# AnimatedRNG/alphazero-rs

Hardware: AMD Instinct MI355X
Metric: selfplay_games_per_sec (higher is better)
Workload: dtype bf16

## Files before the change

alphazero-rs_amd/csrc/az_engine.hip:

```cpp
#include "../../include/az_engine.h"

#include <dlfcn.h>
#include <unistd.h>
#include <rccl/rccl.h>

#include <algorithm>
#include <array>
#include <atomic>
#include <chrono>
#include <cstdio>
#include <cstring>
#include <map>
#include <memory>
#include <mutex>
#include <string>
#include <vector>

#include "az_combine.h"
#include "az_local_comm.h"
#include "az_net.h"
#include "az_train.h"
#include "az_tree.h"

using namespace az;
// ... 917 lines not shown
        const bool eps = is("root_noise_eps_e6");
        if (eps ? (value < 0 || value > 1000000) : (value < 50000 || value > 100000000))
            return fail(e, AZ_ERR_BAD_ARGUMENT, eps ? "root_noise_eps_e6 must be in 0 .. 1000000" : "root_noise_alpha_e6 must be in 50000 .. 100000000");
        if (e->sp_session) return fail(e, AZ_ERR_BAD_ARGUMENT, "root noise cannot change while a self-play session is open");
        (eps ? e->root_noise_eps_e6 : e->root_noise_alpha_e6) = value;
        return AZ_OK;
    }
    if (is("playout_cap_sims") || is("playout_cap_full_e6")) {
        const bool sims = is("playout_cap_sims");
        if (value < 0 || value > (sims ? PLAYOUT_CAP_MAX_SIMS : PLAYOUT_CAP_E6))
            return fail(e, AZ_ERR_BAD_ARGUMENT, sims ? "playout_cap_sims must be in 0 .. 65535" : "playout_cap_full_e6 must be in 0 .. 1000000");
        if (e->sp_session) return fail(e, AZ_ERR_BAD_ARGUMENT, "the playout cap cannot change while a self-play session is open");
        (sims ? e->playout_cap_sims : e->playout_cap_full_e6) = value;
        return AZ_OK;
    }
    if (is("forced_playouts_k_e6") || is("policy_prune")) {
        const bool k = is("forced_playouts_k_e6");
        if (value < 0 || value > (k ? FORCED_K_E6_MAX : 1))
            return fail(e, AZ_ERR_BAD_ARGUMENT, k ? "forced_playouts_k_e6 must be in 0 .. 16000000" : "policy_prune must be 0 or 1");
        if (e->sp_session) return fail(e, AZ_ERR_BAD_ARGUMENT, "forced playouts cannot change while a self-play session is open");
        (k ? e->forced_playouts_k_e6 : e->policy_prune) = value;
        return AZ_OK;
    }
    if (is("arena_opening_plies")) {
        if (value < 0 || value > OPENING_MAX_PLIES || (value & 1)) return fail(e, AZ_ERR_BAD_ARGUMENT, "arena_opening_plies must be 0 or an even value in 2 .. 12");
        e->arena_opening_plies = value;
        return AZ_OK;
    }
    if (is("conv3_small") && (value == 0 || value == 1)) { e->netopt.conv3_small = (int)value; return AZ_OK; }
    if (is("conv3_tail") && (value == 0 || value == 1)) { e->netopt.conv3_tail = (int)value; return AZ_OK; }
    if (is("ring_packed") && (value == 0 || value == 1)) { e->netopt.ring_packed = (int)value; return AZ_OK; }
    if (is("conv3_planes") && (value == 0 || value == 1)) { e->netopt.conv3_planes = (int)value; return AZ_OK; }
    if (is("conv3_wreg") && (value == 0 || value == 1)) { e->netopt.conv3_wreg = (int)value; return AZ_OK; }
    if (is("narrow_rows") && value >= 0 && value <= 65536) { e->netopt.narrow_rows = (int)value; return AZ_OK; }
    if (is("tree_block4") && (value == 0 || value == 1)) { e->tree_block4 = (int)value; return AZ_OK; }
    if (is("dedup_stats") && (value == 0 || value == 1)) { e->dedup_stats = (int)value; return AZ_OK; }
    if (is("profile_every") && value >= 1 && value <= 1000000) { e->profile_every = (int)value; return AZ_OK; }
    if (is("profile") && (value == 0 || value == 1)) { e->prof.on = value != 0; return AZ_OK; }
    if (is("search_graph") && value >= 0 && value <= 1000 && value % 2 == 0) { e->search_graph = (int)value; return AZ_OK; }
    if (is("search_graph_rows") && value >= 0 && value <= 1000000) { e->search_graph_rows = (int)value; return AZ_OK; }
    if (is("selfplay_async") && (value == 0 || value == 1)) { e->selfplay_async = (int)value; return AZ_OK; }
    if (is("selfplay_async_launches") && value >= 1 && value <= 8) { e->selfplay_async_launches = (int)value; return AZ_OK; }
    if (is("selfplay_async_iters") && value >= 2 && value <= 64) { e->selfplay_async_iters = (int)value; return AZ_OK; }
    if (is("fused_search") && (value == 0 || value == 1)) { e->fused_search = (int)value; return AZ_OK; }
    if (is("eval_dedup") && value >= 0 && value <= 2) { e->eval_dedup = (int)value; return AZ_OK; }
    if (is("eval_cache_log2") && (value == 0 || (value >= 10 && value <= 30))) { e->eval_cache_log2 = (int)value; return AZ_OK; }
    if (is("eval_cache_max_stones") && value >= 0 && value <= 42) { e->eval_cache_max_stones = (int)value; return AZ_OK; }
    if (is("eval_cache_persist") && (value == 0 || value == 1)) { e->eval_cache_persist = (int)value; return AZ_OK; }
    if (is("train_epochs") && value >= 1 && value <= 100000) { e->train_epochs = (int)value; return AZ_OK; }
    if (is("train_batch") && value >= 2 && value <= TRAIN_MAX_BATCH) { e->train_batch = (int)value; return AZ_OK; }
    if (is("train_seed")) { e->train_seed = (uint64_t)value; return AZ_OK; }
    if (is("train_graph") && (value == 0 || value == 1)) { e->train_graph = (int)value; if (e->trainer) trainer_set_graph(e->trainer, value != 0); return AZ_OK; }
    if (is("train_gemm3_ring") && (value == 0 || value == 1)) { e->train_gemm3_ring = (int)value; if (e->trainer) trainer_set_gemm3_ring(e->trainer, value != 0); return AZ_OK; }
    if (is("train_fwd_x3") && (value == 0 || value == 1)) { e->train_fwd_x3 = (int)value; if (e->trainer) trainer_set_fwd_x3(e->trainer, value != 0); return AZ_OK; }
    if (is("train_wgrad_tr") && (value == 0 || value == 1)) { e->train_wgrad_tr = (int)value; if (e->trainer) trainer_set_wgrad_tr(e->trainer, value != 0); return AZ_OK; }
    if (is("train_implicit") && (value == 0 || value == 1)) { e->train_implicit = (int)value; if (e->trainer) trainer_set_implicit(e->trainer, value != 0); return AZ_OK; }
    if (is("train_fork") && (value == 0 || value == 1)) {
        e->train_fork = (int)value;
        if (e->trainer) { (void)hipSetDevice(e->device); trainer_set_fork(e->trainer, value != 0); }
        return AZ_OK;
    }
    if (is("train_gemm") && (value == 0 || value == 1)) { e->train_gemm = (int)value; if (e->trainer) trainer_set_gemm(e->trainer, (int)value); return AZ_OK; }
    if (is("train_fwd_dma") && (value == 0 || value == 1)) { e->train_fwd_dma = (int)value; if (e->trainer) trainer_set_fwd_dma(e->trainer, value != 0); return AZ_OK; }
    if (is("train_lr_e9") && value > 0) { e->hyper.lr = (float)((double)value * 1e-9); return AZ_OK; }
    if (is("train_dropout_e6") && value >= 0 && value < 1000000) { e->hyper.dropout = (float)((double)value * 1e-6); return AZ_OK; }
#ifdef AZ_DIAG
// ... 1606 lines not shown
```

alphazero-rs_amd/csrc/az_net.h:

```cpp
#pragma once
#include "az_tree.h"

namespace az {

struct ConvNet;
struct NetWorkspace;

struct Layout {
    int C;
    int64_t conv_w[4], conv_b[4], conv_bn[4], fc_w[2], fc_b[2], fc_bn[2], pi_w, pi_b, v_w, v_b, total;
    explicit Layout(int c) : C(c) {
        int64_t o = 0;
        for (int l = 0; l < 4; ++l) {
            int cin = l == 0 ? 2 : C;
            conv_w[l] = o; o += 9ll * cin * C;
            conv_b[l] = o; o += C;
            conv_bn[l] = o; o += 4ll * C;
        }
        const int fin[2] = {6 * C, 1024}, fout[2] = {1024, 512};
        for (int l = 0; l < 2; ++l) {
            fc_w[l] = o; o += (int64_t)fin[l] * fout[l];
            fc_b[l] = o; o += fout[l];
            fc_bn[l] = o; o += 4ll * fout[l];
        }
// ... 3 lines not shown
    }
};


struct NetProfile {
    double conv2_ms = 0, conv2_flops = 0, total_ms = 0, total_flops = 0;
    double conv3_ms = 0, conv3_flops = 0;
    double conv4_ms = 0, conv4_flops = 0;
    double fc_ms = 0, fc_flops = 0;
    double rows = 0;
    double conv2_bytes = 0;
    uint64_t launches = 0;
};

void launch_net_fixture(const EvalBatch& eb, int kind, uint64_t salt, hipStream_t s);

ConvNet* convnet_create(int channels, const char** err);
void convnet_destroy(ConvNet* n);
NetWorkspace* netws_create(int channels, int max_batch, const char** err);
void netws_destroy(NetWorkspace* ws);
int64_t convnet_param_count(int channels);
bool convnet_set_params(ConvNet* n, const float* host_params, int64_t count);
bool convnet_get_params(const ConvNet* n, float* host_params, int64_t count);
void convnet_init_random(ConvNet* n, uint64_t seed);
void netws_resolve_profile(NetWorkspace* ws, NetProfile* prof);
bool netws_conv3_accounting(NetWorkspace* ws, unsigned long long out[2], bool reset);
struct NetOptions {
    int conv2_table = 1;
    int conv3_small = 1;
    int conv3_planes = 1;
    int ring_packed = 1;
    int conv3_tail = 1;
    int conv3_wreg = 1;
    int net_fp8 = 0;
    int narrow_rows = 32;
    int gemm_variant = 5;
    int conv1_table = 1;
    int conv2_pipe = 1;
    int conv3_pipe = 1;
    int conv3_ring = 0;
    int conv4_big = 0;
    int fc_ring = 1;
    int ring_tile[6] = {0, 0, 0, 0, 0, 0};
};
bool netws_read_clock_stamps(NetWorkspace* ws, unsigned long long* out2048);
long long netws_read_conv3_out(NetWorkspace* ws, int rows, void* out);
#ifdef AZ_DIAG
long long netws_read_act(NetWorkspace* ws, int layer, int rows, void* out);
long long convnet_read_conv_table(const ConvNet* n, int which, int first_row, int n_rows, void* out);
#endif
long long netws_read_conv3_out_fp8(NetWorkspace* ws, int rows, void* out);
long long netws_read_conv2_out_fp8(NetWorkspace* ws, int rows, void* out);
unsigned long long netws_fp8_skinny_launches(const NetWorkspace* ws);
bool convnet_build_fp8(ConvNet* n, NetWorkspace* ws, hipStream_t s);
bool convnet_fp8_scales(const ConvNet* n, float out[2]);
bool convnet_prepare(NetWorkspace* ws, const NetOptions& opt);
void convnet_forward(ConvNet* n, NetWorkspace* ws, const EvalBatch& eb, int n_rows_hint, int n_rows_typ, hipStream_t s, NetProfile* prof,
                     const NetOptions& opt);

}
```

alphazero-rs_amd/csrc/az_net.hip:

```cpp
#include "az_net.h"
#include "az_fp8.h"

#include <algorithm>
#include <cmath>
#include <cstring>
#include <vector>

namespace az {

constexpr int ACTIONS = ConnectFour::ACTIONS;

typedef __bf16 bf16x8 __attribute__((ext_vector_type(8)));
typedef float f32x4 __attribute__((ext_vector_type(4)));
typedef int i32x4 __attribute__((ext_vector_type(4)));
typedef int i32x8 __attribute__((ext_vector_type(8)));

__global__ void k_net_fixture(EvalBatch eb, int kind, uint64_t salt) {
    uint32_t i = blockIdx.x * blockDim.x + threadIdx.x;
    if (i >= *eb.n) return;
    float pi[ACTIONS], v;
    if (kind == 0) {
#pragma unroll
        for (int a = 0; a < ACTIONS; ++a) pi[a] = __fdiv_rn(1.0f, 7.0f);
        v = 1.0f;
// ... 511 lines not shown
    constexpr int BMAX = NS == 2 ? 192 : 128;
    __shared__ __attribute__((aligned(16))) unsigned char smem[NS * (BMAX * 128 + 16384)];
    const int M = (int)(*d.n_dev) * d.rows_per_sample;
    if (M <= d.m_min || (d.m_hi > 0 && M > d.m_hi)) return;
    const int bm = __builtin_amdgcn_readfirstlane(ring_pick_bm(M, d.N / GBN, NS, d.tap_w > 1));
    if constexpr (NS == 2) {
        if (bm == 96) gemm_ring_body<2, 96>(d, smem, M);
        else if (bm == 160) gemm_ring_body<2, 160>(d, smem, M);
        else if (bm == 192) gemm_ring_body<2, 192>(d, smem, M);
        else gemm_ring_body<2, 128>(d, smem, M);
    } else {
        if (bm == 64) gemm_ring_body<4, 64>(d, smem, M);
        else if (bm == 96) gemm_ring_body<4, 96>(d, smem, M);
        else gemm_ring_body<4, 128>(d, smem, M);
    }
}

template <int LAYER, int NS, int F8>
__global__ __launch_bounds__(256, (NS <= 2 ? 2 : 1)) void k_gemm_ring_f8(const GemmDesc d) {
    constexpr int BMAX = NS == 2 ? 192 : 128;
    __shared__ __attribute__((aligned(16))) unsigned char smem[NS * (BMAX * 128 + 16384)];
    const int M = (int)(*d.n_dev) * d.rows_per_sample;
    if (M <= d.m_min) return;
    const int bm = __builtin_amdgcn_readfirstlane(ring_pick_bm(M, d.N / GBN, NS, true));
    if constexpr (NS == 2) {
        if (bm == 96) gemm_ring_body<2, 96, F8>(d, smem, M);
        else if (bm == 160) gemm_ring_body<2, 160, F8>(d, smem, M);
        else if (bm == 192) gemm_ring_body<2, 192, F8>(d, smem, M);
        else gemm_ring_body<2, 128, F8>(d, smem, M);
    } else {
        if (bm == 64) gemm_ring_body<4, 64, F8>(d, smem, M);
        else if (bm == 96) gemm_ring_body<4, 96, F8>(d, smem, M);
        else gemm_ring_body<4, 128, F8>(d, smem, M);
    }
}

constexpr int HBN_ = 256;
constexpr int HBN2_ = 128;
constexpr int IMG_NB = 6;
constexpr int IMG_ROWS = IMG_NB * 42;
constexpr int IMG_ZERO_ROW = 252;

__device__ __forceinline__ void lds_dma16(const void* sbase, uint32_t voff, uint32_t lds_addr);
template <int LAYER, bool TABLE = false>
__global__ __launch_bounds__(256, 2) void k_conv_same_pipe(const GemmDesc d) {
    __shared__ __attribute__((aligned(16))) unsigned char smem[2 * 32768];
    const int n_boards = (int)(*d.n_dev);
    const int M = n_boards * 42;
    const int C = d.cin;
    const int NT = d.N / HBN2_;
    const int id = blockIdx.x;
    const int xcd = id & 7, j = id >> 3;
    const int ntile = j % NT, mtile = (j / NT) * 8 + xcd;
    const int b0 = mtile * IMG_NB, n0 = ntile * HBN2_;
    if (b0 >= n_boards) return;
    const int tid = threadIdx.x, lane = tid & 63;
    const int wave = __builtin_amdgcn_readfirstlane(tid >> 6);
    const int wr = wave >> 1, wc = wave & 1;
    if (tid < 8) *(uint4*)(smem + IMG_ZERO_ROW * 128 + tid * 16) = make_uint4(0, 0, 0, 0);
    const int lrow = lane >> 3;
    const int chunk = (lane & 7) ^ lrow;
    uint32_t i_ob[8];
#pragma unroll
    for (int q = 0; q < 8; ++q) {
        int r = (q * 4 + wave) * 8 + lrow;
        r = r < IMG_ROWS ? r : IMG_ROWS - 1;
// ... 133 lines not shown
            for (int nt = 0; nt < 4; ++nt) {
                const int nl = wc * 64 + nt * 16 + fq * 4;
                const float4 bv = *(const float4*)(d.bias + n0 + nl);
#pragma unroll
                for (int mt = 0; mt < 8; ++mt) {
                    const int rl = mt * 16 + frow;
                    float r0 = acc[mt][nt][0] + bv.x, r1 = acc[mt][nt][1] + bv.y, r2 = acc[mt][nt][2] + bv.z,
                          r3 = acc[mt][nt][3] + bv.w;
                    if (d.relu) { r0 = fmaxf(r0, 0.f); r1 = fmaxf(r1, 0.f); r2 = fmaxf(r2, 0.f); r3 = fmaxf(r3, 0.f); }
                    uint2 o;
                    o.x = pack_bf16x2(r0, r1);
                    o.y = pack_bf16x2(r2, r3);
                    *(uint2*)(smem + rl * EP_STRIDE + nl * 2) = o;
                }
            }
        }
        __syncthreads();
#pragma unroll
        for (int it = 0; it < 128 * 16 / 256; ++it) {
            const int idx = it * 256 + tid;
            const int rl = idx >> 4, c = idx & 15;
            const int ml = half * 128 + rl;
            const int m = b0 * 42 + ml;
            if (ml >= IMG_ROWS || m >= M) continue;
            *(uint4*)(d.out + (size_t)m * d.N + n0 + c * 8) = *(const uint4*)(smem + rl * EP_STRIDE + c * 16);
        }
        __syncthreads();
    }
}

constexpr int C3_PLANE_BYTES = 32768;
constexpr int C3_TAB_INV = 512;
constexpr int C3_TAB_RD = 9 * 2 * 16 * 8;
constexpr int WF3_STEP = 4096;
constexpr int WF3_PAD = 1;
constexpr int C3_NB = 12;

template <int NB, int IH, int IW, int MT, int NTW, bool PLANES = false, int WREG = 0>
struct ConvTile {
    static constexpr int OH = IH - 2, OW = IW - 2, OUT_PER = OH * OW, IN_PER = IH * IW;
    static constexpr int OUT_ROWS = NB * OUT_PER, IMG_R = NB * IN_PER;
    static constexpr int NCOL = 32 * NTW, WROWS = 16 * MT;
    static constexpr int IMG_BYTES = PLANES ? 2 * C3_PLANE_BYTES : (IMG_R * 128 + 1023) / 1024 * 1024;
    static constexpr int LDS_BYTES = IMG_BYTES + (WREG ? 0 : NCOL * 128);
    static constexpr int EP_STRIDE = NCOL * 2 + 16;
    static_assert(OUT_ROWS <= 2 * WROWS && IMG_R % 8 == 0 && MT % 2 == 0, "tile");
    static_assert(LDS_BYTES <= 81920, "two workgroups must fit a CU's 160 KiB");
    static_assert(OUT_ROWS * EP_STRIDE <= LDS_BYTES, "the output tile must fit the dead buffers");
};

template <int NB, int IH, int IW, int MT, int NTW, bool PLANES = false, int WREG = 0>
__device__ __forceinline__ void conv_valid_tile(const GemmDesc& d, unsigned char* smem, const int b0 , const int n0 ,
                                                const int n_boards) {
    using T = ConvTile<NB, IH, IW, MT, NTW, PLANES, WREG>;
    static_assert(!PLANES || (NB == C3_NB && IH == 6 && IW == 7 && MT == 8), "the cell maps are conv3's");
    constexpr int OUT_PER = T::OUT_PER, IN_PER = T::IN_PER, OUT_ROWS = T::OUT_ROWS, IMG_R = T::IMG_R, NCOL = T::NCOL, OW = T::OW;
    constexpr int IMG_BYTES = T::IMG_BYTES;
    constexpr int IPIECES = (IMG_R + 31) / 32, WPIECES = NCOL / 32;
    constexpr int MH = MT / 2;
    constexpr int NM = MH * NTW;
    const int M = n_boards * OUT_PER;
    const int C = d.cin;
    const int tid = threadIdx.x, lane = tid & 63;
    const int wave = __builtin_amdgcn_readfirstlane(tid >> 6);
    const int wr = wave >> 1, wc = wave & 1;
    const int lrow = lane >> 3;
    const int chunk = (lane & 7) ^ lrow;
    typedef __attribute__((address_space(3))) void* lds_ptr;
// ... 478 lines not shown
        float s = xf[0] * w0.x + xf[1] * w0.y + xf[2] * w0.z + xf[3] * w0.w + xf[4] * w1.x + xf[5] * w1.y + xf[6] * w1.z +
                  xf[7] * w1.w;
#pragma unroll
        for (int off = 32; off >= 1; off >>= 1) s += __shfl_xor(s, off, 64);
        o[k] = s + bias[k];
    }
    if (lane == 0) {
        float mx = o[0];
#pragma unroll
        for (int a = 1; a < ACTIONS; ++a) mx = fmaxf(mx, o[a]);
        float e[ACTIONS], sum = 0.f;
#pragma unroll
        for (int a = 0; a < ACTIONS; ++a) { e[a] = expf(o[a] - mx); sum += e[a]; }
#pragma unroll
        for (int a = 0; a < ACTIONS; ++a) eb.pi[(size_t)wave * 8 + a] = e[a] / sum;
        const float vv = tanhf(o[7]);
        eb.pi[(size_t)wave * 8 + 7] = vv;
        eb.v[wave] = vv;
    }
}

struct ConvNet {
    int C = 512;
    std::vector<float> params;
    std::vector<void*> dev;
    float *w1 = nullptr, *b1 = nullptr;
    uint16_t* t1 = nullptr;
    uint16_t* u2 = nullptr;
    uint16_t* w2r = nullptr;
    uint32_t* npat = nullptr;
    uint16_t* wg[5] = {nullptr};
    uint16_t* wr[5] = {nullptr};
    uint16_t* wf3 = nullptr;
    float* bg[5] = {nullptr};
    float *wh = nullptr, *bh = nullptr;
    unsigned char* w8[2] = {nullptr, nullptr};
    float* dq8[2] = {nullptr, nullptr};
    float sa2 = 0.f, sa3 = 0.f;
    bool fp8_ready = false;
    template <class T> T* dalloc(size_t n) {
        void* p = nullptr;
        if (hipMalloc(&p, n * sizeof(T)) != hipSuccess) return nullptr;
        dev.push_back(p);
        return (T*)p;
    }
};

static std::vector<uint16_t> conv3_tables() {
    constexpr int NB = C3_NB, IH = 6, IW = 7, OW = 5, OUT_PER = 20, IN_PER = 42;
    std::vector<uint16_t> t((size_t)C3_TAB_INV + C3_TAB_RD, 0);
    int next_m[4] = {0, 0, 0, 0};
    std::vector<int> cell(NB * IN_PER, 0);
    for (int bl = 0; bl < NB; ++bl)
        for (int y = 0; y < IH; ++y)
            for (int x = 0; x < IW; ++x) {
                const int label = (OUT_PER * bl + OW * y + x) & 15, cls = label >> 2, h2 = label & 3;
                const int rho = 4 * next_m[cls]++ + cls;
                if (rho >= C3_TAB_INV) return {};
                const int r = bl * IN_PER + y * IW + x;
                t[rho] = (uint16_t)(r | (h2 << 10));
                cell[r] = rho * 64 + h2 * 16;
            }
    for (int tap = 0; tap < 9; ++tap)
        for (int wr = 0; wr < 2; ++wr)
            for (int frow = 0; frow < 16; ++frow)
                for (int mt = 0; mt < 8; ++mt) {
// ... 24 lines not shown
        if (hipMalloc(&p, n * sizeof(T)) != hipSuccess) return nullptr;
        dev.push_back(p);
        return (T*)p;
    }
};

int64_t convnet_param_count(int channels) { return Layout(channels).total; }

ConvNet* convnet_create(int channels, const char** err) {
    if (channels % 128 != 0 || channels < 128) { if (err) *err = "net_channels must be a multiple of 128"; return nullptr; }
    ConvNet* n = new ConvNet();
    n->C = channels;
    const int C = channels;
    bool ok = true;
    ok &= (n->w1 = n->dalloc<float>(18 * (size_t)C)) != nullptr;
    ok &= (n->b1 = n->dalloc<float>(C)) != nullptr;
    ok &= (n->t1 = n->dalloc<uint16_t>((size_t)CONV1_PATTERNS * C)) != nullptr;
    ok &= (n->u2 = n->dalloc<uint16_t>((size_t)(CONV1_PATTERNS + 1) * 9 * C)) != nullptr;
    if (n->u2) ok &= hipMemset(n->u2 + (size_t)CONV1_PATTERNS * 9 * C, 0, (size_t)9 * C * sizeof(uint16_t)) == hipSuccess;
    ok &= (n->w2r = n->dalloc<uint16_t>((size_t)9 * C * C)) != nullptr;
    ok &= (n->npat = n->dalloc<uint32_t>(1)) != nullptr;
    if (ok) { const uint32_t np = CONV1_PATTERNS; ok = hipMemcpy(n->npat, &np, sizeof np, hipMemcpyHostToDevice) == hipSuccess; }
    const size_t wk[5] = {9 * (size_t)C, 9 * (size_t)C, 9 * (size_t)C, 6 * (size_t)C, 1024};
    const size_t wn[5] = {(size_t)C, (size_t)C, (size_t)C, 1024, 512};
    for (int l = 0; l < 5; ++l) {
        ok &= (n->wg[l] = n->dalloc<uint16_t>(wk[l] * wn[l])) != nullptr;
        ok &= (n->bg[l] = n->dalloc<float>(wn[l])) != nullptr;
        if (l >= 1) ok &= (n->wr[l] = n->dalloc<uint16_t>(wk[l] * wn[l])) != nullptr;
    }
    ok &= (n->wh = n->dalloc<float>(8 * 512)) != nullptr;
    ok &= (n->bh = n->dalloc<float>(8)) != nullptr;
    ok &= (n->wf3 = n->dalloc<uint16_t>(9 * (size_t)C * C + (size_t)WF3_PAD * WF3_STEP)) != nullptr;
    if (n->wf3) ok &= hipMemset(n->wf3 + 9 * (size_t)C * C, 0, (size_t)WF3_PAD * WF3_STEP * sizeof(uint16_t)) == hipSuccess;
    if (!ok) {
        if (err) *err = "convnet_create: device allocation failed";
        convnet_destroy(n);
        return nullptr;
    }
    return n;
}

void convnet_destroy(ConvNet* n) {
    if (!n) return;
    for (void* p : n->dev) (void)hipFree(p);
    delete n;
}

NetWorkspace* netws_create(int channels, int max_batch, const char** err) {
    NetWorkspace* n = new NetWorkspace();
    n->C = channels;
    n->max_batch = max_batch;
    const int C = channels;
    const size_t B = (size_t)max_batch;
    bool ok = true;
    ok &= (n->act2 = n->dalloc<uint16_t>((B + 16) * 42 * C)) != nullptr;
    ok &= (n->act3 = n->dalloc<uint16_t>(B * 20 * C)) != nullptr;
    ok &= (n->act4 = n->dalloc<uint16_t>(B * 6 * C)) != nullptr;
    ok &= (n->fc1o = n->dalloc<uint16_t>(B * 1024)) != nullptr;
    ok &= (n->fc2o = n->dalloc<uint16_t>(B * 512)) != nullptr;
    ok &= (n->dbg = n->dalloc<unsigned long long>(2048)) != nullptr;
    if (ok) ok = hipMemset(n->dbg, 0, 2048 * 8) == hipSuccess;
    ok &= (n->acct = n->dalloc<unsigned long long>(2)) != nullptr;
    if (ok) ok = hipMemset(n->acct, 0, 16) == hipSuccess;
    ok &= (n->c3tab = n->dalloc<uint16_t>(C3_TAB_INV + C3_TAB_RD)) != nullptr;
    if (ok) {
        const std::vector<uint16_t> tab = conv3_tables();
// ... 58 lines not shown
        ok &= hipMemcpy(net->w1, w.data(), w.size() * 4, hipMemcpyHostToDevice) == hipSuccess;
        ok &= hipMemcpy(net->b1, b.data(), b.size() * 4, hipMemcpyHostToDevice) == hipSuccess;
        hipLaunchKernelGGL(k_conv1_table, dim3(CONV1_PATTERNS), dim3(64), 0, nullptr, net->w1, net->b1, net->t1, C);
        ok &= hipDeviceSynchronize() == hipSuccess;
    }
    const int64_t w_off[5] = {L.conv_w[1], L.conv_w[2], L.conv_w[3], L.fc_w[0], L.fc_w[1]};
    const int64_t b_off[5] = {L.conv_b[1], L.conv_b[2], L.conv_b[3], L.fc_b[0], L.fc_b[1]};
    const int64_t bn_off[5] = {L.conv_bn[1], L.conv_bn[2], L.conv_bn[3], L.fc_bn[0], L.fc_bn[1]};
    const int K[5] = {9 * C, 9 * C, 9 * C, 6 * C, 1024}, N[5] = {C, C, C, 1024, 512};
    for (int l = 0; l < 5; ++l) {
        std::vector<uint16_t> w((size_t)K[l] * N[l]);
        std::vector<float> b(N[l]);
        for (int nn = 0; nn < N[l]; ++nn) {
            float s, t;
            fold_scale(p + bn_off[l], N[l], nn, &s, &t);
            b[nn] = p[b_off[l] + nn] * s + t;
            for (int k = 0; k < K[l]; ++k) w[(size_t)nn * K[l] + k] = f32_to_bf16_host(p[w_off[l] + (int64_t)k * N[l] + nn] * s);
        }
        ok &= hipMemcpy(net->wg[l], w.data(), w.size() * 2, hipMemcpyHostToDevice) == hipSuccess;
        ok &= hipMemcpy(net->bg[l], b.data(), b.size() * 4, hipMemcpyHostToDevice) == hipSuccess;
        if (net->wr[l]) {
            std::vector<uint16_t> wr(w.size());
            const int cin = l <= 2 ? C : K[l], ntaps = K[l] / cin, nk = K[l] / 64;
            for (int nt = 0; nt < N[l] / 128; ++nt)
                for (int kt = 0; kt < nk; ++kt) {
                    const int cb = kt / ntaps, tap = kt - cb * ntaps, kk = tap * cin + cb * 64;
                    uint16_t* img = &wr[((size_t)nt * nk + kt) * 8192];
                    for (int r = 0; r < 128; ++r)
                        for (int sl = 0; sl < 8; ++sl)
                            std::memcpy(img + r * 64 + sl * 8, &w[(size_t)(nt * 128 + r) * K[l] + kk + ((sl ^ (r & 7)) << 3)], 16);
                }
            ok &= hipMemcpy(net->wr[l], wr.data(), wr.size() * 2, hipMemcpyHostToDevice) == hipSuccess;
        }
        if (l == 1 && net->wf3) {
            std::vector<uint16_t> wf((size_t)9 * C * C);
            const int nk = C / 64 * 9;
            for (int g = 0; g < C / 64; ++g)
                for (int kt = 0; kt < nk; ++kt) {
                    const int cb = kt / 9, tap = kt - cb * 9;
                    uint16_t* st = &wf[((size_t)g * nk + kt) * WF3_STEP];
                    for (int j = 0; j < 4; ++j)
                        for (int ks = 0; ks < 2; ++ks)
                            for (int ln = 0; ln < 64; ++ln) {
                                const int frow = ln & 15, fq = ln >> 4;
                                std::memcpy(st + ((j * 2 + ks) * 64 + ln) * 8,
                                            &w[(size_t)(g * 64 + j * 16 + frow) * K[1] + (size_t)tap * C + cb * 64 + ks * 32 + fq * 8], 16);
                            }
                }
            ok &= hipMemcpy(net->wf3, wf.data(), wf.size() * 2, hipMemcpyHostToDevice) == hipSuccess;
        }
        if (l == 0) {
            std::vector<uint16_t> wr((size_t)9 * C * C);
            for (int co = 0; co < C; ++co)
                for (int t = 0; t < 9; ++t)
                    std::memcpy(&wr[((size_t)t * C + co) * C], &w[(size_t)co * K[0] + (size_t)t * C], (size_t)C * 2);
            ok &= hipMemcpy(net->w2r, wr.data(), wr.size() * 2, hipMemcpyHostToDevice) == hipSuccess;
            GemmDesc d{};
            d.A = net->t1; d.W = net->w2r; d.bias = net->bg[0]; d.out = net->u2; d.n_dev = net->npat;
            d.rows_per_sample = 1; d.out_w = 1; d.in_h = 1; d.in_w = 1; d.in_c = C; d.tap_w = 1; d.cin = C; d.K = C; d.N = 9 * C;
            d.relu = 0; d.out_f16 = 1;
            const int mt8 = ((CONV1_PATTERNS + GBM - 1) / GBM + 7) / 8 * 8;
            hipLaunchKernelGGL(k_gemm_mfma<6>, dim3(mt8 * (d.N / GBN)), dim3(256), 0, nullptr, d);
            ok &= hipDeviceSynchronize() == hipSuccess;
        }
    }
    {
        std::vector<float> w(8 * 512), b(8);
        for (int k = 0; k < 512; ++k) {
            for (int a = 0; a < 7; ++a) w[(size_t)a * 512 + k] = p[L.pi_w + (int64_t)k * 7 + a];
            w[(size_t)7 * 512 + k] = p[L.v_w + k];
        }
        for (int a = 0; a < 7; ++a) b[a] = p[L.pi_b + a];
        b[7] = p[L.v_b];
        ok &= hipMemcpy(net->wh, w.data(), w.size() * 4, hipMemcpyHostToDevice) == hipSuccess;
        ok &= hipMemcpy(net->bh, b.data(), b.size() * 4, hipMemcpyHostToDevice) == hipSuccess;
    }
    return ok;
}

bool convnet_get_params(const ConvNet* n, float* host_params, int64_t count) {
    if (!n || (int64_t)n->params.size() != count) return false;
    std::memcpy(host_params, n->params.data(), (size_t)count * sizeof(float));
// ... 19 lines not shown
    for (int l = 0; l < 4; ++l) {
        int cin = l == 0 ? 2 : C;
        fill(L.conv_w[l], 9ll * cin * C, 9 * cin, 9 * C);
        bn_default(L.conv_bn[l], C);
    }
    fill(L.fc_w[0], 6ll * C * 1024, 6 * C, 1024); bn_default(L.fc_bn[0], 1024);
    fill(L.fc_w[1], 1024ll * 512, 1024, 512); bn_default(L.fc_bn[1], 512);
    fill(L.pi_w, 512 * 7, 512, 7);
    fill(L.v_w, 512, 512, 1);
    convnet_set_params(net, p.data(), L.total);
}


static bool conv3_is_small(const GemmDesc& d, int rows_hint, int rows_typ) {
    return (rows_typ > 0 ? (long long)rows_typ * 115 / 100 : (long long)rows_hint) * d.rows_per_sample <= 8192;
}
template <bool TABLE>
static void launch_conv2_gemm(const GemmDesc& d, int rows_hint, hipStream_t s) {
    const int tiles = (rows_hint + IMG_NB - 1) / IMG_NB;
    const int t8 = (tiles + 7) / 8 * 8;
    hipLaunchKernelGGL((k_conv_same_pipe<1, TABLE>), dim3(t8 * (d.N / HBN2_)), dim3(256), 0, s, d);
}
static void launch_conv3_image(const GemmDesc& d, int rows_hint, hipStream_t s, bool tail, bool planes, bool wreg) {
    const int tiles = (rows_hint + C3_NB - 1) / C3_NB;
    const int t8 = (tiles + 7) / 8 * 8;
    const int full_grid = t8 * (d.N / 128), tail_wgs = tail ? C3_TAIL : 0;
    const dim3 grid(full_grid + tail_wgs), block(256);
    if (wreg && planes && d.Wf) hipLaunchKernelGGL((k_conv3_auto_wreg<2>), grid, block, 0, s, d, full_grid, tail_wgs);
    else if (planes) hipLaunchKernelGGL((k_conv3_auto<2, true>), grid, block, 0, s, d, full_grid, tail_wgs);
    else hipLaunchKernelGGL((k_conv3_auto<2, false>), grid, block, 0, s, d, full_grid, tail_wgs);
}

template <int LAYER, int F8 = 0>
static void launch_ring_auto(const GemmDesc& d, int rows_hint, int rows_typ, hipStream_t s, bool force_one_per_cu = false) {
    const int m_est = (int)((rows_typ > 0 ? (long long)rows_typ * 115 / 100 : (long long)rows_hint) * d.rows_per_sample), ncol = d.N / GBN;
    const bool conv = d.tap_w > 1;
    const int tile_max = conv ? 96 : 128;
    const int m_one = 256 / ncol * tile_max;
    const int m_bound = rows_hint * d.rows_per_sample;
    auto launch = [&](bool one_per_cu, const GemmDesc& dd, int m_cover) {
        const int bmin = one_per_cu ? 64 : 96;
        const int mtb = ((m_cover + bmin - 1) / bmin + 7) / 8 * 8;
        if constexpr (F8 != 0) {
            if (one_per_cu) hipLaunchKernelGGL((k_gemm_ring_f8<LAYER, 4, F8>), dim3(mtb * ncol), dim3(256), 0, s, dd);
            else hipLaunchKernelGGL((k_gemm_ring_f8<LAYER, 2, F8>), dim3(mtb * ncol), dim3(256), 0, s, dd);
        } else if (one_per_cu) hipLaunchKernelGGL((k_gemm_ring_auto<LAYER, 4>), dim3(mtb * ncol), dim3(256), 0, s, dd);
        else hipLaunchKernelGGL((k_gemm_ring_auto<LAYER, 2>), dim3(mtb * ncol), dim3(256), 0, s, dd);
    };
    if (!force_one_per_cu && !conv && m_bound > m_one && (long long)m_est * 100 >= (long long)m_one * 70 && (long long)m_est * 100 <= (long long)m_one * 140) {
        GemmDesc lo = d, hi = d;
        lo.m_hi = m_one;
        hi.m_min = std::max(d.m_min, m_one);
        launch(true, lo, std::min(m_bound, m_one));
        launch(false, hi, m_bound);
        return;
    }
    const bool one_per_cu = force_one_per_cu || m_bound <= m_one || (m_est + tile_max - 1) / tile_max * ncol <= 256;
    launch(one_per_cu, d, m_bound);
}

#ifdef AZ_DIAG
template <int LAYER>
static bool launch_gemm_diag(const GemmDesc& d, int rows_hint, int rows_typ, hipStream_t s, const NetOptions& o) {
    const int v = o.gemm_variant;
    if ((v == 3 || v == 5) && LAYER == 1 && d.N % HBN_ == 0 && d.cin % 64 == 0) {
        const int tiles = (rows_hint + IMG_NB - 1) / IMG_NB;
        const int t8 = (tiles + 7) / 8 * 8;
        if (v == 5 && o.conv2_pipe) return false;
        if (v == 5 && d.states) hipLaunchKernelGGL((k_conv_img2<LAYER, true>), dim3(t8 * (d.N / HBN2_)), dim3(256), 0, s, d);
        else if (v == 5) hipLaunchKernelGGL((k_conv_img2<LAYER>), dim3(t8 * (d.N / HBN2_)), dim3(256), 0, s, d);
        else hipLaunchKernelGGL((k_conv_img<LAYER>), dim3(t8 * (d.N / HBN_)), dim3(512), 0, s, d);
        return true;
    }
    const bool big = v >= 1 && (LAYER == 1 || LAYER == 2 || (LAYER == 3 && !o.ring_tile[3] && (o.conv4_big == 1 || (o.conv4_big == 2 && rows_typ >= 4096)))) &&
                     d.N % HBN_ == 0;
    if constexpr (LAYER == 2) if (v == 5 && o.conv3_ring) {
        const int mt = (rows_hint * d.rows_per_sample + GBM - 1) / GBM;
        const int mt8 = (mt + 7) / 8 * 8;
// ... 74 lines not shown
template <int LAYER>
static void launch_gemm(const GemmDesc& d, int rows_hint, int rows_typ, hipStream_t s, const NetOptions& o) {
#ifdef AZ_DIAG
    if (launch_gemm_diag<LAYER>(d, rows_hint, rows_typ, s, o)) return;
#endif
    GemmDesc dd = d;
    if constexpr (LAYER >= 2) if (o.narrow_rows > 0 && d.N % 32 == 0) {
        const int lim = o.narrow_rows * (LAYER == 2 ? 1 : LAYER == 3 ? 2 : 4);
        const int est = rows_typ > 0 ? rows_typ : rows_hint;
        if (est <= 16 * lim) {
            dd.m_max = lim * d.rows_per_sample;
            const int rows_cov = rows_hint < lim ? rows_hint : lim;
            const dim3 grid((unsigned)skinny_waves_max(rows_cov * d.rows_per_sample, d.N)), block(64);
            const int nk = d.K / GBK;
            if (nk % 8 == 0) hipLaunchKernelGGL((k_gemm_skinny<LAYER, 8>), grid, block, 0, s, dd);
            else if (nk % 6 == 0) hipLaunchKernelGGL((k_gemm_skinny<LAYER, 6>), grid, block, 0, s, dd);
            else hipLaunchKernelGGL((k_gemm_skinny<LAYER, 2>), grid, block, 0, s, dd);
            if (rows_hint <= lim) return;
            dd.m_min = dd.m_max;
        }
    }
    const GemmDesc& d2 = dd;
    if constexpr (LAYER == 1) if (d.N % HBN_ == 0 && d.cin % 64 == 0) {
        if (d.states) launch_conv2_gemm<true>(d2, rows_hint, s);
        else launch_conv2_gemm<false>(d2, rows_hint, s);
        return;
    }
    if constexpr (LAYER == 2) {
        if (o.conv3_small && conv3_is_small(d2, rows_hint, rows_typ)) launch_ring_auto<LAYER>(d2, rows_hint, rows_typ, s, true);
        else launch_conv3_image(d2, rows_hint, s, o.conv3_tail != 0, o.conv3_planes != 0, o.conv3_wreg != 0);
        return;
    }

    launch_ring_auto<LAYER>(d2, rows_hint, rows_typ, s);
}

template <int LAYER, int F8>
static void launch_gemm_f8(const GemmDesc& d, int rows_hint, int rows_typ, hipStream_t s, const NetOptions& o, NetWorkspace* ws) {
    GemmDesc dd = d;
    if (o.narrow_rows > 0 && d.N % 32 == 0 && d.cin % 128 == 0) {
        const int lim = o.narrow_rows * (LAYER == 2 ? 1 : 2);
        const int est = rows_typ > 0 ? rows_typ : rows_hint;
        if (est <= 16 * lim) {
            dd.m_max = lim * d.rows_per_sample;
            const int rows_cov = rows_hint < lim ? rows_hint : lim;
            const dim3 grid((unsigned)skinny_waves_max(rows_cov * d.rows_per_sample, d.N)), block(64);
            const int nk = d.K / 128;
            if (nk % 18 == 0) hipLaunchKernelGGL((k_gemm_skinny_f8<LAYER, F8, 9, 6>), grid, block, 0, s, dd);
            else hipLaunchKernelGGL((k_gemm_skinny_f8<LAYER, F8, 9, 3>), grid, block, 0, s, dd);
            ++ws->fp8_skinny_launches;
            if (rows_hint <= lim) return;
            dd.m_min = dd.m_max;
        }
    }
    launch_ring_auto<LAYER, F8>(dd, rows_hint, rows_typ, s);
}

unsigned long long netws_fp8_skinny_launches(const NetWorkspace* n) { return n ? n->fp8_skinny_launches : 0; }

static hipEvent_t net_event(NetWorkspace* n) {
    if (!n->ev_pool.empty()) { hipEvent_t e = n->ev_pool.back(); n->ev_pool.pop_back(); return e; }
    hipEvent_t e = nullptr;
    (void)hipEventCreate(&e);
    return e;
}

bool netws_conv3_accounting(NetWorkspace* n, unsigned long long out[2], bool reset) {
// ... 241 lines not shown
    d.acct = ws->acct;
    d.A = table ? n->t1 : ws->act1; d.states = table ? eb.state : nullptr;
    d.W = n->wg[0]; d.bias = n->bg[0]; d.out = ws->act2;
    d.rows_per_sample = 42; d.out_w = 7; d.in_h = 8; d.in_w = 9; d.in_c = C; d.tap_w = 3; d.cin = C; d.K = 9 * C; d.N = C;
    if (timed) (void)hipEventRecord(rec.e1, s);
    if (table2) {
#ifdef AZ_DIAG
        if (o.conv2_table == 2) {
            const size_t blocks = std::min<size_t>(((size_t)rows_hint * 6 + 3) / 4, 256 * 8);
            hipLaunchKernelGGL(k_conv2_table, dim3((unsigned)blocks), dim3(256), (size_t)9 * C * 2, s, eb, n->u2, n->bg[0], ws->act2, C);
        } else
#endif
        {
            const size_t nsl = (size_t)C / 64;
            const size_t blocks = std::min<size_t>(((size_t)rows_hint + 3) / 4, 256) * nsl;
            if (fp8) hipLaunchKernelGGL(k_conv2_table_x8, dim3((unsigned)blocks), dim3(256), 0, s, eb, n->u2, n->bg[0], ws->act2, C, n->sa2);
            else hipLaunchKernelGGL(k_conv2_table_x, dim3((unsigned)blocks), dim3(256), 0, s, eb, n->u2, n->bg[0], ws->act2, C);
        }
    } else {
        launch_gemm<1>(d, rows_hint, rows_typ, s, o);
    }
    if (timed) (void)hipEventRecord(rec.e2, s);
    d.states = nullptr;
    d.A = ws->act2; d.W = n->wg[1]; d.bias = n->bg[1]; d.out = ws->act3;
    d.rows_per_sample = 20; d.out_w = 5; d.in_h = 6; d.in_w = 7;
    d.Wr = o.ring_packed ? n->wr[1] : nullptr;
    d.Wf = n->wf3;
    if (fp8) {
        GemmDesc d8 = d;
        d8.Wr = (const uint16_t*)n->w8[0]; d8.dq = n->dq8[0]; d8.out_scale = n->sa3; d8.Wf = nullptr;
        launch_gemm_f8<2, 1>(d8, rows_hint, rows_typ, s, o, ws);
    } else
    launch_gemm<2>(d, rows_hint, rows_typ, s, o);
    d.Wf = nullptr;
    if (timed) (void)hipEventRecord(rec.e2b, s);
    d.A = ws->act3; d.W = n->wg[2]; d.bias = n->bg[2]; d.out = ws->act4;
    d.Wr = o.ring_packed ? n->wr[2] : nullptr;
    d.rows_per_sample = 6; d.out_w = 3; d.in_h = 4; d.in_w = 5;
    if (fp8) {
        GemmDesc d8 = d;
        d8.Wr = (const uint16_t*)n->w8[1]; d8.dq = n->dq8[1];
        launch_gemm_f8<3, 2>(d8, rows_hint, rows_typ, s, o, ws);
    } else
    launch_gemm<3>(d, rows_hint, rows_typ, s, o);
    if (timed) (void)hipEventRecord(rec.e2c, s);
    d.A = ws->act4; d.W = n->wg[3]; d.bias = n->bg[3]; d.out = ws->fc1o;
    d.Wr = o.ring_packed ? n->wr[3] : nullptr;
    d.rows_per_sample = 1; d.out_w = 1; d.in_h = 1; d.in_w = 1; d.in_c = 6 * C; d.tap_w = 1; d.cin = 6 * C; d.K = 6 * C; d.N = 1024;
    launch_gemm<4>(d, rows_hint, rows_typ, s, o);
    d.A = ws->fc1o; d.W = n->wg[4]; d.bias = n->bg[4]; d.out = ws->fc2o;
    d.Wr = o.ring_packed ? n->wr[4] : nullptr;
    d.in_c = 1024; d.cin = 1024; d.K = 1024; d.N = 512;
    launch_gemm<5>(d, rows_hint, rows_typ, s, o);
    hipLaunchKernelGGL(k_heads, dim3((rows_hint * 64 + 255) / 256), dim3(256), 0, s, eb, ws->fc2o, n->wh, n->bh, n_log);
    if (timed) {
        (void)hipEventRecord(rec.e3, s);
        ws->open.push_back(rec);
    }
}

}
```

Before: 10060.

## Add ring GEMM variant that streams MFMA-packed weights directly into registers

Adds a new ring-pipelined GEMM kernel in which the B (weight) operand is loaded with buffer loads straight into registers in a pre-swizzled fragment layout, while only the activation tile is staged through LDS via DMA. Fragment-packed weight copies are built for conv4, fc1 and fc2, generalising the existing conv3 packing, and the ring launcher uses this kernel when the new default-on ring_wreg option is set and a packed buffer exists. The aim is to cut LDS traffic and LDS capacity spent on weights and to free LDS for deeper stages or larger M tiles. In exchange it uses more VGPRs for the in-flight weight fragments, relies on hand-tuned vmcnt waits, and allocates extra device memory for the packed weights.

```diff
diff --git a/alphazero-rs_amd/csrc/az_engine.hip b/alphazero-rs_amd/csrc/az_engine.hip
--- a/alphazero-rs_amd/csrc/az_engine.hip
+++ b/alphazero-rs_amd/csrc/az_engine.hip
@@ -973,6 +973,7 @@
     if (is("ring_packed") && (value == 0 || value == 1)) { e->netopt.ring_packed = (int)value; return AZ_OK; }
     if (is("conv3_planes") && (value == 0 || value == 1)) { e->netopt.conv3_planes = (int)value; return AZ_OK; }
     if (is("conv3_wreg") && (value == 0 || value == 1)) { e->netopt.conv3_wreg = (int)value; return AZ_OK; }
+    if (is("ring_wreg") && (value == 0 || value == 1)) { e->netopt.ring_wreg = (int)value; return AZ_OK; }
     if (is("narrow_rows") && value >= 0 && value <= 65536) { e->netopt.narrow_rows = (int)value; return AZ_OK; }
     if (is("tree_block4") && (value == 0 || value == 1)) { e->tree_block4 = (int)value; return AZ_OK; }
     if (is("dedup_stats") && (value == 0 || value == 1)) { e->dedup_stats = (int)value; return AZ_OK; }
diff --git a/alphazero-rs_amd/csrc/az_net.h b/alphazero-rs_amd/csrc/az_net.h
--- a/alphazero-rs_amd/csrc/az_net.h
+++ b/alphazero-rs_amd/csrc/az_net.h
@@ -59,6 +59,7 @@
     int ring_packed = 1;
     int conv3_tail = 1;
     int conv3_wreg = 1;
+    int ring_wreg = 1;
     int net_fp8 = 0;
     int narrow_rows = 32;
     int gemm_variant = 5;
diff --git a/alphazero-rs_amd/csrc/az_net.hip b/alphazero-rs_amd/csrc/az_net.hip
--- a/alphazero-rs_amd/csrc/az_net.hip
+++ b/alphazero-rs_amd/csrc/az_net.hip
@@ -567,6 +567,163 @@
         if (bm == 64) gemm_ring_body<4, 64, F8>(d, smem, M);
         else if (bm == 96) gemm_ring_body<4, 96, F8>(d, smem, M);
         else gemm_ring_body<4, 128, F8>(d, smem, M);
+    }
+}
+
+constexpr int WF3_STEP = 4096;
+constexpr int WF3_PAD = 1;
+
+template <int Y, int NLD>
+__device__ __forceinline__ void ring_wait_younger(const int younger) {
+    if (younger >= Y) asm volatile("s_waitcnt vmcnt(%0)" ::"n"(Y * NLD) : "memory");
+    else if constexpr (Y > 0) ring_wait_younger<Y - 1, NLD>(younger);
+}
+template <int NS, int BM>
+__device__ __forceinline__ void gemm_ring_wreg_body(const GemmDesc& d, unsigned char* smem , const int M) {
+    static_assert(BM % 32 == 0 && BM >= 64 && BM <= 192 && NS >= 3 && NS * BM * 128 <= 163840 && (NS - 2) * (BM / 32 + 4) <= 63, "tile");
+    constexpr int MT = BM / 32;
+    constexpr int MF = BM / 16;
+    constexpr int STAGE = BM * 128;
+    constexpr int NLD = MT + 4;
+    const int ntaps = d.K / d.cin;
+    const int NT = d.N / GBN;
+    const int id = blockIdx.x;
+    const int xcd = id & 7, j = id >> 3;
+    const int ntile = j % NT, mtile = (j / NT) * 8 + xcd;
+    const int m0 = mtile * BM, n0 = ntile * GBN;
+    if (m0 >= M) return;
+    const int tid = threadIdx.x, lane = tid & 63;
+    const int wave = __builtin_amdgcn_readfirstlane(tid >> 6);
+    const int lrow = lane >> 3;
+    const int chunk = (lane & 7) ^ lrow;
+    uint32_t a_ob[MT];
+#pragma unroll
+    for (int q = 0; q < MT; ++q) {
+        int m = m0 + (q * 4 + wave) * 8 + lrow;
+        m = m < M ? m : M - 1;
+        const int b = m / d.rows_per_sample, r = m - b * d.rows_per_sample;
+        const int y = r / d.out_w, x = r - y * d.out_w;
+        a_ob[q] = (uint32_t)(((b * d.in_h + y) * d.in_w + x) * d.in_c + chunk * 8) * 2u;
+    }
+    typedef __attribute__((address_space(3))) void* lds_ptr;
+    const uint32_t lds0 = (uint32_t)(uintptr_t)(lds_ptr)(smem + wave * 1024);
+    const int nk = d.K / GBK;
+    const __amdgpu_buffer_rsrc_t wrs = __builtin_amdgcn_make_buffer_rsrc((void*)d.Wf, 0, (d.K * d.N + WF3_PAD * WF3_STEP) * 2, 0x00020000);
+    uint32_t wfo = (uint32_t)(((n0 >> 6) + (wave >> 1)) * nk) * 8192u + (uint32_t)((wave & 1) * 2) * 2048u;
+    const uint32_t wlane = (uint32_t)lane * 16u;
+    i32x4 fw[NS][4];
+    int ks_tap = 0, ks_kx = 0;
+    uint32_t ks_c0 = 0, ks_toff = 0;
+#define AZ_WLD(dst_, imm_) \
+    asm volatile("buffer_load_dwordx4 %0, %1, %2, %3 offen offset:%4" : "=v"(dst_) : "v"(wlane), "s"(wrs), "s"(wfo), "n"(imm_) : "memory")
+#define AZ_RISSUE(buf_)                                                                                 \
+    {                                                                                                   \
+        const char* abase = (const char*)d.A + (size_t)ks_toff * 2;                                     \
+        const uint32_t la = lds0 + (buf_) * STAGE;                                                      \
+        _Pragma("unroll") for (int q_ = 0; q_ < MT; ++q_) lds_dma16(abase, a_ob[q_], la + q_ * 4096);   \
+        AZ_WLD(fw[buf_][0], 0); AZ_WLD(fw[buf_][1], 2048); AZ_WLD(fw[buf_][2], 1024); AZ_WLD(fw[buf_][3], 3072); \
+        wfo += 8192u;                                                                                   \
+        ++ks_tap; ++ks_kx; ks_toff += (uint32_t)d.in_c;                                                 \
+        if (ks_kx == d.tap_w) { ks_kx = 0; ks_toff += (uint32_t)((d.in_w - d.tap_w) * d.in_c); }        \
+        if (ks_tap == ntaps) { ks_tap = 0; ks_kx = 0; ks_c0 += GBK; ks_toff = ks_c0; }                  \
+    }
+    f32x4 acc[MF][2];
+#pragma unroll
+    for (int i = 0; i < MF; ++i)
+#pragma unroll
+        for (int jn = 0; jn < 2; ++jn) acc[i][jn] = f32x4{0.f, 0.f, 0.f, 0.f};
+    const int frow = lane & 15, fq = lane >> 4, fsw = lane & 7;
+    const int coff0 = ((0 + fq) ^ fsw) << 4, coff1 = ((4 + fq) ^ fsw) << 4;
+#pragma unroll
+    for (int st = 0; st < NS - 1; ++st)
+        if (st < nk) AZ_RISSUE(st);
+#define AZ_RSTEP(S_)                                                                                    \
+    if (kt < nk) {                                                                                      \
+         \
+        ring_wait_younger<NS - 2, NLD>(nk - 1 - kt);                                                    \
+        asm volatile("" : "+v"(fw[S_][0]), "+v"(fw[S_][1]), "+v"(fw[S_][2]), "+v"(fw[S_][3]));          \
+        __builtin_amdgcn_s_barrier();                     \
+        __builtin_amdgcn_sched_barrier(0);                                                              \
+        if (kt + NS - 1 < nk) AZ_RISSUE((S_ + NS - 1) % NS);                                            \
+        __builtin_amdgcn_sched_barrier(0);                                                              \
+        const unsigned char* sA = smem + (S_) * STAGE;                                                  \
+        bf16x8 fa0[MF], fa1[MF];                                                                        \
+        _Pragma("unroll") for (int mt = 0; mt < MF; ++mt) fa0[mt] = *(const bf16x8*)(sA + (mt * 16 + frow) * 128 + coff0); \
+        _Pragma("unroll") for (int mt = 0; mt < MF; ++mt) fa1[mt] = *(const bf16x8*)(sA + (mt * 16 + frow) * 128 + coff1); \
+        _Pragma("unroll") for (int mt = 0; mt < MF; ++mt)                                               \
+            _Pragma("unroll") for (int nt = 0; nt < 2; ++nt)                                            \
+                acc[mt][nt] = __builtin_amdgcn_mfma_f32_16x16x32_bf16(__builtin_bit_cast(bf16x8, fw[S_][nt]), fa0[mt], acc[mt][nt], 0, 0, 0); \
+        _Pragma("unroll") for (int mt = 0; mt < MF; ++mt)                                               \
+            _Pragma("unroll") for (int nt = 0; nt < 2; ++nt)                                            \
+                acc[mt][nt] = __builtin_amdgcn_mfma_f32_16x16x32_bf16(__builtin_bit_cast(bf16x8, fw[S_][2 + nt]), fa1[mt], acc[mt][nt], 0, 0, 0); \
+         \
+        __builtin_amdgcn_sched_group_barrier(0x100, MF, 0);                                             \
+        _Pragma("unroll") for (int g = 0; g < MF; ++g) {                                                \
+            __builtin_amdgcn_sched_group_barrier(0x008, 2, 0);                                          \
+            __builtin_amdgcn_sched_group_barrier(0x100, 1, 0);                                          \
+        }                                                                                               \
+        __builtin_amdgcn_sched_group_barrier(0x008, 2 * MF, 0);                                         \
+        __builtin_amdgcn_sched_barrier(0);                                                              \
+        ++kt;                                                                                           \
+    }
+    for (int kt = 0; kt < nk;) {
+        AZ_RSTEP(0);
+        AZ_RSTEP(1);
+        AZ_RSTEP(2);
+        if constexpr (NS > 3) AZ_RSTEP(3);
+        if constexpr (NS > 4) { AZ_RSTEP(4); AZ_RSTEP(5); }
+        if constexpr (NS > 6) { AZ_RSTEP(6); AZ_RSTEP(7); }
+    }
+#undef AZ_RSTEP
+#undef AZ_RISSUE
+#undef AZ_WLD
+    constexpr int EP_STRIDE = 272;
+    static_assert(BM * EP_STRIDE <= NS * STAGE, "the output tile must fit the ring");
+    __builtin_amdgcn_s_waitcnt(0xC07F);
+    __builtin_amdgcn_s_barrier();
+#pragma unroll
+    for (int nt = 0; nt < 2; ++nt) {
+        const int nl = wave * 32 + nt * 16 + fq * 4;
+        const float4 bv = *(const float4*)(d.bias + n0 + nl);
+#pragma unroll
+        for (int mt = 0; mt < MF; ++mt) {
+            const int ml = mt * 16 + frow;
+            float r0 = acc[mt][nt][0] + bv.x, r1 = acc[mt][nt][1] + bv.y, r2 = acc[mt][nt][2] + bv.z, r3 = acc[mt][nt][3] + bv.w;
+            if (d.relu) { r0 = fmaxf(r0, 0.f); r1 = fmaxf(r1, 0.f); r2 = fmaxf(r2, 0.f); r3 = fmaxf(r3, 0.f); }
+            uint2 o;
+            o.x = pack_bf16x2(r0, r1);
+            o.y = pack_bf16x2(r2, r3);
+            *(uint2*)(smem + ml * EP_STRIDE + nl * 2) = o;
+        }
+    }
+    __syncthreads();
+#pragma unroll
+    for (int it = 0; it < BM * 16 / 256; ++it) {
+        const int idx = it * 256 + tid;
+        const int ml = idx / 16, c = idx % 16;
+        const int m = m0 + ml;
+        if (m >= M) continue;
+        *(uint4*)((unsigned char*)d.out + ((size_t)m * d.N + n0) * 2 + c * 16) = *(const uint4*)(smem + ml * EP_STRIDE + c * 16);
+    }
+}
+
+template <int LAYER, int NS, bool TWO>
+__global__ __launch_bounds__(256, (TWO ? 2 : 1)) void k_gemm_ring_wreg(const GemmDesc d) {
+    __shared__ __attribute__((aligned(16))) unsigned char smem[TWO ? 4 * 160 * 128 : NS * 128 * 128];
+    const int M = (int)(*d.n_dev) * d.rows_per_sample;
+    if (M <= d.m_min || (d.m_hi > 0 && M > d.m_hi)) return;
+    const int bm = __builtin_amdgcn_readfirstlane(ring_pick_bm(M, d.N / GBN, TWO ? 2 : 4, d.tap_w > 1));
+    if constexpr (TWO) {
+        if (bm == 96) gemm_ring_wreg_body<4, 96>(d, smem, M);
+        else if (bm == 160) gemm_ring_wreg_body<4, 160>(d, smem, M);
+        else if (bm == 192) {
+            if ((M + 191) / 192 * (d.N / GBN) <= 512) gemm_ring_body<2, 192>(d, smem, M);
+            else gemm_ring_wreg_body<3, 192>(d, smem, M);
+        } else gemm_ring_wreg_body<4, 128>(d, smem, M);
+    } else {
+        if (bm == 64) gemm_ring_wreg_body<NS, 64>(d, smem, M);
+        else if (bm == 96) gemm_ring_wreg_body<NS, 96>(d, smem, M);
+        else gemm_ring_wreg_body<NS, 128>(d, smem, M);
     }
 }
 
@@ -766,8 +923,6 @@
 constexpr int C3_PLANE_BYTES = 32768;
 constexpr int C3_TAB_INV = 512;
 constexpr int C3_TAB_RD = 9 * 2 * 16 * 8;
-constexpr int WF3_STEP = 4096;
-constexpr int WF3_PAD = 1;
 constexpr int C3_NB = 12;
 
 template <int NB, int IH, int IW, int MT, int NTW, bool PLANES = false, int WREG = 0>
@@ -1312,6 +1467,7 @@
     uint16_t* wg[5] = {nullptr};
     uint16_t* wr[5] = {nullptr};
     uint16_t* wf3 = nullptr;
+    uint16_t* wf[5] = {nullptr};
     float* bg[5] = {nullptr};
     float *wh = nullptr, *bh = nullptr;
     unsigned char* w8[2] = {nullptr, nullptr};
@@ -1402,6 +1558,11 @@
     ok &= (n->bh = n->dalloc<float>(8)) != nullptr;
     ok &= (n->wf3 = n->dalloc<uint16_t>(9 * (size_t)C * C + (size_t)WF3_PAD * WF3_STEP)) != nullptr;
     if (n->wf3) ok &= hipMemset(n->wf3 + 9 * (size_t)C * C, 0, (size_t)WF3_PAD * WF3_STEP * sizeof(uint16_t)) == hipSuccess;
+    n->wf[1] = n->wf3;
+    for (int l = 2; l < 5; ++l) {
+        ok &= (n->wf[l] = n->dalloc<uint16_t>(wk[l] * wn[l] + (size_t)WF3_PAD * WF3_STEP)) != nullptr;
+        if (n->wf[l]) ok &= hipMemset(n->wf[l] + wk[l] * wn[l], 0, (size_t)WF3_PAD * WF3_STEP * sizeof(uint16_t)) == hipSuccess;
+    }
     if (!ok) {
         if (err) *err = "convnet_create: device allocation failed";
         convnet_destroy(n);
@@ -1526,22 +1687,21 @@
                 }
             ok &= hipMemcpy(net->wr[l], wr.data(), wr.size() * 2, hipMemcpyHostToDevice) == hipSuccess;
         }
-        if (l == 1 && net->wf3) {
-            std::vector<uint16_t> wf((size_t)9 * C * C);
-            const int nk = C / 64 * 9;
-            for (int g = 0; g < C / 64; ++g)
+        if (net->wf[l]) {
+            std::vector<uint16_t> wf(w.size());
+            const int cin = l <= 2 ? C : K[l], ntaps = K[l] / cin, nk = K[l] / 64;
+            for (int g = 0; g < N[l] / 64; ++g)
                 for (int kt = 0; kt < nk; ++kt) {
-                    const int cb = kt / 9, tap = kt - cb * 9;
+                    const int cb = kt / ntaps, tap = kt - cb * ntaps, kk = tap * cin + cb * 64;
                     uint16_t* st = &wf[((size_t)g * nk + kt) * WF3_STEP];
                     for (int j = 0; j < 4; ++j)
                         for (int ks = 0; ks < 2; ++ks)
                             for (int ln = 0; ln < 64; ++ln) {
                                 const int frow = ln & 15, fq = ln >> 4;
-                                std::memcpy(st + ((j * 2 + ks) * 64 + ln) * 8,
-                                            &w[(size_t)(g * 64 + j * 16 + frow) * K[1] + (size_t)tap * C + cb * 64 + ks * 32 + fq * 8], 16);
+                                std::memcpy(st + ((j * 2 + ks) * 64 + ln) * 8, &w[(size_t)(g * 64 + j * 16 + frow) * K[l] + kk + ks * 32 + fq * 8], 16);
                             }
                 }
-            ok &= hipMemcpy(net->wf3, wf.data(), wf.size() * 2, hipMemcpyHostToDevice) == hipSuccess;
+            ok &= hipMemcpy(net->wf[l], wf.data(), wf.size() * 2, hipMemcpyHostToDevice) == hipSuccess;
         }
         if (l == 0) {
             std::vector<uint16_t> wr((size_t)9 * C * C);
@@ -1627,7 +1787,7 @@
 }
 
 template <int LAYER, int F8 = 0>
-static void launch_ring_auto(const GemmDesc& d, int rows_hint, int rows_typ, hipStream_t s, bool force_one_per_cu = false) {
+static void launch_ring_auto(const GemmDesc& d, int rows_hint, int rows_typ, hipStream_t s, bool force_one_per_cu = false, bool wreg = false) {
     const int m_est = (int)((rows_typ > 0 ? (long long)rows_typ * 115 / 100 : (long long)rows_hint) * d.rows_per_sample), ncol = d.N / GBN;
     const bool conv = d.tap_w > 1;
     const int tile_max = conv ? 96 : 128;
@@ -1639,6 +1799,9 @@
         if constexpr (F8 != 0) {
             if (one_per_cu) hipLaunchKernelGGL((k_gemm_ring_f8<LAYER, 4, F8>), dim3(mtb * ncol), dim3(256), 0, s, dd);
             else hipLaunchKernelGGL((k_gemm_ring_f8<LAYER, 2, F8>), dim3(mtb * ncol), dim3(256), 0, s, dd);
+        } else if (wreg && dd.Wf) {
+            if (one_per_cu) hipLaunchKernelGGL((k_gemm_ring_wreg<LAYER, 4, false>), dim3(mtb * ncol), dim3(256), 0, s, dd);
+            else hipLaunchKernelGGL((k_gemm_ring_wreg<LAYER, 4, true>), dim3(mtb * ncol), dim3(256), 0, s, dd);
         } else if (one_per_cu) hipLaunchKernelGGL((k_gemm_ring_auto<LAYER, 4>), dim3(mtb * ncol), dim3(256), 0, s, dd);
         else hipLaunchKernelGGL((k_gemm_ring_auto<LAYER, 2>), dim3(mtb * ncol), dim3(256), 0, s, dd);
     };
@@ -1779,7 +1942,7 @@
         return;
     }
 
-    launch_ring_auto<LAYER>(d2, rows_hint, rows_typ, s);
+    launch_ring_auto<LAYER>(d2, rows_hint, rows_typ, s, false, o.ring_wreg != 0);
 }
 
 template <int LAYER, int F8>
@@ -2087,10 +2250,10 @@
         launch_gemm_f8<2, 1>(d8, rows_hint, rows_typ, s, o, ws);
     } else
     launch_gemm<2>(d, rows_hint, rows_typ, s, o);
-    d.Wf = nullptr;
     if (timed) (void)hipEventRecord(rec.e2b, s);
     d.A = ws->act3; d.W = n->wg[2]; d.bias = n->bg[2]; d.out = ws->act4;
     d.Wr = o.ring_packed ? n->wr[2] : nullptr;
+    d.Wf = n->wf[2];
     d.rows_per_sample = 6; d.out_w = 3; d.in_h = 4; d.in_w = 5;
     if (fp8) {
         GemmDesc d8 = d;
@@ -2101,10 +2264,12 @@
     if (timed) (void)hipEventRecord(rec.e2c, s);
     d.A = ws->act4; d.W = n->wg[3]; d.bias = n->bg[3]; d.out = ws->fc1o;
     d.Wr = o.ring_packed ? n->wr[3] : nullptr;
+    d.Wf = n->wf[3];
     d.rows_per_sample = 1; d.out_w = 1; d.in_h = 1; d.in_w = 1; d.in_c = 6 * C; d.tap_w = 1; d.cin = 6 * C; d.K = 6 * C; d.N = 1024;
     launch_gemm<4>(d, rows_hint, rows_typ, s, o);
     d.A = ws->fc1o; d.W = n->wg[4]; d.bias = n->bg[4]; d.out = ws->fc2o;
     d.Wr = o.ring_packed ? n->wr[4] : nullptr;
+    d.Wf = n->wf[4];
     d.in_c = 1024; d.cin = 1024; d.K = 1024; d.N = 512;
     launch_gemm<5>(d, rows_hint, rows_typ, s, o);
     hipLaunchKernelGGL(k_heads, dim3((rows_hint * 64 + 255) / 256), dim3(256), 0, s, eb, ws->fc2o, n->wh, n->bh, n_log);
```

Result: faster. 10190, median of 6 (+1.3%).
